# EyalMichaeli/SaSPA-Aug

Hardware: AMD Instinct MI355X
Metric: augmented images/sec (512x512, 50-step DDIM) (higher is better)
Workload: dtype bf16; 1 GPU; SD-v1.5 + Canny ControlNet, batch=8 512x512, 50 DDIM steps, CFG 7.5, ctrl-scale 0.75 (BASELINE.json configs[1]); step = Canny + CLIP + 50x(UNet+ControlNet) + VAE decode; batch_per_gpu=8, resolution=512, ddim_steps=50, weights=random-init, architecture-exact, parallelism=dp1 (image shards, one RCCL gather of the status vector), process_group=none (single process)

## Files before the change

### saspa-aug_amd/csrc/gemm_internal.h

```cpp
#pragma once
#include <hip/hip_runtime.h>

#include "saspa_hip.h"

__attribute__((visibility("hidden"))) int saspa_gemm_pp_launch(const SaspaGemmParams& p, hipStream_t s, int ksplit, int fn);
__attribute__((visibility("hidden"))) bool saspa_gemm_pp_eligible(const SaspaGemmParams& p);
__attribute__((visibility("hidden"))) int saspa_gemm_splitk_reduce(const SaspaGemmParams& p, hipStream_t s, int ksplit);
__attribute__((visibility("hidden"))) int saspa_gemm_npart8(const SaspaGemmParams& p, int BM, int BN, int G, int tiles);
static inline int saspa_balanced_grid(int tiles, int cap) {
  if (cap < 1) cap = 1;
  if (tiles <= cap) return tiles;
  const int rounds = (tiles + cap - 1) / cap;
  return (tiles + rounds - 1) / rounds;
}

__attribute__((visibility("hidden"))) int saspa_gemm_ws_launch(const SaspaGemmParams& p, hipStream_t s);
__attribute__((visibility("hidden"))) bool saspa_gemm_ws_eligible(const SaspaGemmParams& p);
__attribute__((visibility("hidden"))) int saspa_gemm_as_launch(const SaspaGemmParams& p, hipStream_t s);
__attribute__((visibility("hidden"))) bool saspa_gemm_as_ok(const SaspaGemmParams& p);
__attribute__((visibility("hidden"))) int saspa_gn_slabs(int c8);
```

### saspa-aug_amd/csrc/saspa_gemm_pp.hip

```cpp
#include <cstdlib>

#include "common.h"
#include "gemm_internal.h"

#ifndef SASPA_PP_CT_ABL
#define SASPA_PP_CT_ABL 0
#endif

namespace {

typedef bf16_t T;

__device__ __forceinline__ void mma(const u32x4& wf, const u32x4& xf, f32x4& acc) {
  acc = __builtin_amdgcn_mfma_f32_16x16x32_bf16(__builtin_bit_cast(bf16x8, wf), __builtin_bit_cast(bf16x8, xf), acc, 0, 0, 0);
}

template <int N> __device__ __forceinline__ void wait_vm() { asm volatile("s_waitcnt vmcnt(%0)" ::"n"(N) : "memory"); }

template <int FN, bool PW, bool UP, int LOOP>
__global__ __launch_bounds__(512) void gemm_pp_kernel(const SaspaGemmParams p, const int ntiles_abl, const int npart8) {
  constexpr bool ONEBAR = LOOP == 1;
  const int ntiles = ntiles_abl & 0x00ffffff;
#ifdef SASPA_GEMM_ABLATION
  const int abl = (ntiles_abl >> 28) & 15;
  const bool stamp = (ntiles_abl >> 27) & 1;
  unsigned long long st0 = 0, sr0 = 0, st1 = 0, sr1 = 0, sr_setup = 0, sr_issue = 0, sr_e0 = 0, sr_e1 = 0;
  const unsigned long long sr_entry = __builtin_amdgcn_s_memrealtime();
  const int eabl = (ntiles_abl >> 24) & 7;
#else
  constexpr int abl = SASPA_PP_CT_ABL, eabl = 0;
#endif
  constexpr int BM = 256, BN = 64 * FN, BK = 64, SZ = 2;
  constexpr int STAGE = (BM + BN) * 8;
  constexpr int CP = BN + 8;
  constexpr int EPI = 128 * CP * SZ / 16;
  constexpr int NLDS = 2 * STAGE > EPI ? 2 * STAGE : EPI;
  constexpr int NIMG = 4;
  constexpr int ADDV_F = (1 + 2 * NIMG) * BN;
  __shared__ u32x4 lds[NLDS + ADDV_F / 4];
  float* const addvb = reinterpret_cast<float*>(lds + NLDS);
  float* const addvr = addvb + BN;

  const int tid = threadIdx.x;
  const int lane = tid & 63;
  const int wave = __builtin_amdgcn_readfirstlane(tid >> 6);
  const int wm = wave >> 2, wn = wave & 3;
  const int frow = lane & 15, fg = lane >> 4;
  const int lr = lane >> 3;
  const int kcs = (lane & 7) ^ lr;

  const int nbn = (p.N + BN - 1) / BN;
  const int G = gridDim.x;
  int tile;
  {
    const int L = blockIdx.x;
    const int qd = G >> 3, rr = G & 7, xcd = L & 7, idx = L >> 3;
    tile = (xcd < rr ? xcd * (qd + 1) : rr * (qd + 1) + (xcd - rr) * qd) + idx;
  }
  const int z = blockIdx.z;
  const int i1 = z / p.nb2, i2 = z - i1 * p.nb2;
  const T* a0 = reinterpret_cast<const T*>(p.a0) + (i1 * p.sa1 + i2 * p.sa2);
  const T* a1 = reinterpret_cast<const T*>(p.a1);
  const T* w = reinterpret_cast<const T*>(p.w) + (i1 * p.sw1 + i2 * p.sw2);
  const long long ooff = i1 * p.so1 + i2 * p.so2;

  const int nk_all = (p.K + BK - 1) / BK;
  const int kt_per = (nk_all + gridDim.y - 1) / gridDim.y;
  const int kt0 = blockIdx.y * kt_per;
  const int nk = max(0, min(nk_all, kt0 + kt_per) - kt0);

  const int hw = p.hout * p.wout;
  const int ctot = p.c0 + p.c1;
  const int chunk_major = p.korder == SASPA_KORDER_CHUNK ? 1 : 0;
  const int hv = UP ? 2 * p.hin : p.hin, wv = UP ? 2 * p.win : p.win;
  const int back = (PW || UP) ? 0 : p.win + 1;
  const T* a0s = a0 - (long long)back * p.lda0;
  const T* a1s = p.c1 > 0 ? a1 - (long long)back * p.lda1 : a0s;
  auto make_desc = [](const T* base, bool live) __attribute__((always_inline)) {
    return __builtin_amdgcn_make_buffer_rsrc(const_cast<T*>(base), (short)0, live ? 0x7fffffff : 0, 0x00020000);
  };
  const rsrc_t rsn = make_desc(w, false);

  int bm = 0, bn = 0;
  int va[4], vb[PW ? 1 : 4], vc[UP ? 4 : 1];
  unsigned offb0 = 0;
  int nrows = 0;
  int ku = 0, cu = 0, dyu = 0, dxu = 0, staged = 0;
  int src = -1;
  const int arow0 = wm * 128 + (wave & 3) * 8 + lr;

  auto setup_tile = [&](int t) __attribute__((always_inline)) {
    if (npart8 > 0) {
      const int G8 = G >> 3;
      const int k = t / G, r = t - k * G;
      const int x = r / G8;
      const int q = k * G8 + (r - x * G8);
      bm = q / npart8;
      bn = x * npart8 + (q - bm * npart8);
    } else {
      bm = t / nbn;
      bn = t - bm * nbn;
    }
    if (!PW) {
      int m = bm * BM + arow0;
      int b = m / hw;
      int rem = m - b * hw;
      int oy = rem / p.wout;
      int ox = rem - oy * p.wout;
#pragma unroll
      for (int s = 0; s < 4; ++s) {
        const bool live = m < p.M;
        const int eb = live ? b : 0, ey = live ? oy : 0, ex = live ? ox : 0;
        const int iy0 = ey * p.stride - p.pad, ix0 = ex * p.stride - p.pad;
        if (UP) {
          va[s] = eb * p.hin * p.win;
          vc[UP ? s : 0] = ((iy0 + 1) << 16) | (ix0 + 1);
          int mask = 0;
          for (int ty = 0; ty < 3; ++ty)
            for (int tx = 0; tx < 3; ++tx)
              if ((unsigned)(iy0 + ty) < (unsigned)hv && (unsigned)(ix0 + tx) < (unsigned)wv) mask |= 1 << (ty * 3 + tx);
          vb[PW ? 0 : s] = mask;
        } else {
          int outside = 0;
#pragma unroll
          for (int tb = 0; tb < 9; ++tb) {
            if (tb == 4) continue;
            const int ty = tb / 3, tx = tb - ty * 3;
            if (!((unsigned)(iy0 + ty) < (unsigned)hv && (unsigned)(ix0 + tx) < (unsigned)wv)) outside |= 1 << (tb < 4 ? tb : tb - 1);
          }
          vb[PW ? 0 : s] = (eb * p.hin * p.win + (ey * p.stride) * p.win + ex * p.stride) | (outside << 24);
        }
        m += 32;
        ox += 32;
        while (ox >= p.wout) { ox -= p.wout; ++oy; }
        while (oy >= p.hout) { oy -= p.hout; ++b; }
      }
    }
    offb0 = (unsigned)((bn * BN + wave * 8 + lr) * p.ldw * SZ + kcs * 16);
    nrows = p.N - bn * BN;
    ku = kt0 * BK;
    if (chunk_major) {
      const int ntap = p.kh * p.kw;
      const int chunk = kt0 / ntap, tap = kt0 - chunk * ntap;
      cu = chunk * BK;
      dyu = tap / p.kw;
      dxu = tap - dyu * p.kw;
    } else {
      const int tapu = ku / ctot;
      cu = ku - tapu * ctot;
      dyu = tapu / p.kw;
      dxu = tapu - dyu * p.kw;
    }
    staged = 0;
    src = -1;
  };

  bool sv = false;
  rsrc_t rs = rsn, rswv = rsn;
  int ldsz = 0, soff = 0, soffw = 0, sdy = 0, sdx = 0, bsh = 0, tapbit = 0;
  unsigned amask = 0;
  auto begin_stage = [&]() __attribute__((always_inline)) {
    sv = staged < nk;
    const bool s0 = cu < p.c0;
    ldsz = (s0 ? p.lda0 : p.lda1) * SZ;
    rs = make_desc(s0 ? a0s : a1s, sv);
    rswv = make_desc(w, sv);
    soff = (s0 ? cu : cu - p.c0) * SZ;
    soffw = ku * SZ;
    if (!UP) {
      if (!ONEBAR && src != (s0 ? 0 : 1)) {
        src = s0 ? 0 : 1;
#pragma unroll
        for (int s = 0; s < 4; ++s) {
          int px;
          if (PW) {
            const int m = bm * BM + arow0 + 32 * s;
            px = m < p.M ? m : 0;
          } else {
            px = vb[PW ? 0 : s] & 0xffffff;
          }
          va[s] = (int)(__umul24((unsigned)px, (unsigned)ldsz) + (unsigned)(kcs * 16));
        }
      }
      if (!PW) {
        const int tb = dyu * 3 + dxu;
        soff += (dyu * p.win + dxu) * ldsz;
        bsh = 7 - (tb < 4 ? tb : tb - 1);
        amask = tb == 4 ? 0u : 0x80000000u;
      }
    } else {
      tapbit = dyu * 3 + dxu;
      sdy = dyu;
      sdx = dxu;
    }
    ++staged;
    ku += BK;
    const int cu_t = cu + BK;
    const int wc = (cu_t >= ctot) ? 1 : 0;
    const int dx1 = dxu + (chunk_major ? 1 : wc);
    const int wx = (dx1 == p.kw) ? 1 : 0;
    const int dy1 = dyu + wx;
    const int wy = (chunk_major && dy1 == p.kh) ? 1 : 0;
    cu = chunk_major ? cu + (wy ? BK : 0) : (wc ? cu_t - ctot : cu_t);
    dxu = wx ? 0 : dx1;
    dyu = wy ? 0 : dy1;
  };
  int cur = 0, oth = STAGE;
  const int swz0 = fg ^ (frow & 7);
  int ra0 = (wm * 128 + frow) * 8 + swz0, ra1 = ra0 ^ 4;
  int rb0 = (BM + wn * (16 * FN) + frow) * 8 + swz0, rb1 = rb0 ^ 4;
  const int dma_a = (wm * 128 + (wave & 3) * 8) * 8;
  const int dma_b = (BM + wave * 8) * 8;

  auto stage_a = [&](const int s, const int buf) __attribute__((always_inline)) {
    unsigned off;
    if (UP) {
      const int iy = ((vc[UP ? s : 0] >> 16) - 1 + sdy) >> 1, ix = ((vc[UP ? s : 0] & 0xffff) - 1 + sdx) >> 1;
      const int px = va[s] + iy * p.win + ix;
      const bool ok = ((vb[PW ? 0 : s] >> tapbit) & 1) != 0;
      off = ok ? __umul24((unsigned)px, (unsigned)ldsz) + (unsigned)(kcs * 16) : kInvalid;
    } else if (PW) {
      if (ONEBAR) {
        const int m = bm * BM + arow0 + 32 * s;
        off = __umul24((unsigned)(m < p.M ? m : 0), (unsigned)ldsz) + (unsigned)(kcs * 16);
      } else {
        off = (unsigned)va[s];
      }
    } else {
      const unsigned base = ONEBAR ? __umul24((unsigned)vb[PW ? 0 : s] & 0xffffffu, (unsigned)ldsz) + (unsigned)(kcs * 16) : (unsigned)va[s];
      off = (((unsigned)vb[PW ? 0 : s] << bsh) & amask) | base;
    }
    __builtin_amdgcn_raw_ptr_buffer_load_lds(rs, (lds_void_t*)(lds + buf + dma_a + s * 32 * 8), 16, (int)off, soff, 0, 0);
  };
  auto stage_b = [&](const int i, const int buf) __attribute__((always_inline)) {
    const bool ok = (wave + 8 * i) * 8 < nrows;
    __builtin_amdgcn_raw_ptr_buffer_load_lds(rswv, (lds_void_t*)(lds + buf + dma_b + i * 64 * 8), 16, (int)(ok ? offb0 : kInvalid),
                                             soffw + i * 64 * p.ldw * SZ, 0, 0);
  };
  auto stage_slice = [&](const int s, const int buf) __attribute__((always_inline)) {
    stage_a(s, buf);
    if (s < 3) {
      stage_b(s, buf);
    } else {
#pragma unroll
      for (int i = 3; i < FN; ++i) stage_b(i, buf);
    }
  };

  f32x4 acc[8][FN];
  u32x4 wb[FN][2], xa[2][2];
  int dbgv[4] = {0, 0, 0, 0};
#if defined(SASPA_GEMM_ABLATION) || SASPA_PP_CT_ABL
#pragma unroll
  for (int j = 0; j < FN; ++j) wb[j][0] = wb[j][1] = u32x4{(unsigned)j, 0u, 0x3f803f80u, 0x3f803f80u};
#pragma unroll
  for (int i = 0; i < 2; ++i) xa[i][0] = xa[i][1] = u32x4{(unsigned)i, 1u, 0x3f803f80u, 0x3f803f80u};
#endif

  auto phase = [&](const int P, const int SS, const int sbuf, const bool sync) __attribute__((always_inline)) {
    if (!(abl & 2)) {
      if (P == 0) {
#pragma unroll
        for (int j = 0; j < FN; ++j) {
          wb[j][0] = lds[rb0 + j * 16 * 8];
          wb[j][1] = lds[rb1 + j * 16 * 8];
        }
        __builtin_amdgcn_sched_barrier(0);
      }
#pragma unroll
      for (int i = 0; i < 2; ++i) {
        xa[i][0] = lds[ra0 + (P * 32 + i * 16) * 8];
        xa[i][1] = lds[ra1 + (P * 32 + i * 16) * 8];
      }
    }
    if (!(abl & 4)) stage_slice(SS, sbuf);
    if (sync && P == 3) wait_vm<6>();
    if (sync && P == 0) asm volatile("s_waitcnt lgkmcnt(4)" ::: "memory");
    if (sync && !(abl & 8)) __builtin_amdgcn_s_barrier();
    __builtin_amdgcn_s_setprio(1);
    if (abl & 1) {
#pragma unroll
      for (int i = 0; i < 2; ++i) { asm volatile("" ::"v"(xa[i][0])); asm volatile("" ::"v"(xa[i][1])); }
#pragma unroll
      for (int j = 0; j < FN; ++j) { asm volatile("" ::"v"(wb[j][0])); asm volatile("" ::"v"(wb[j][1])); }
    } else {
#pragma unroll
      for (int kk = 0; kk < 2; ++kk)
#pragma unroll
        for (int i = 0; i < 2; ++i)
#pragma unroll
          for (int j = 0; j < FN; ++j) mma(wb[j][kk], xa[i][kk], acc[P * 2 + i][j]);
    }
    __builtin_amdgcn_s_setprio(0);
    if (sync && !(abl & 8)) __builtin_amdgcn_s_barrier();
  };

  setup_tile(tile);
#ifdef SASPA_GEMM_ABLATION
  if (stamp) sr_setup = __builtin_amdgcn_s_memrealtime();
#endif
  for (;;) {
#pragma unroll
    for (int i = 0; i < 8; ++i)
#pragma unroll
      for (int j = 0; j < FN; ++j) acc[i][j] = f32x4{0.f, 0.f, 0.f, 0.f};

    if (gridDim.y == 1) {
      constexpr int PCS = BN / 64;
      const int nimg = p.rowvec ? NIMG : 1;
      for (int pc = wave; pc < PCS * (1 + 2 * NIMG); pc += 8) {
        const int rowi = pc / PCS, part = pc - rowi * PCS;
        const int voff = (bn * BN + part * 64 + lane) * 4;
        if (rowi == 0) {
          const rsrc_t rb = __builtin_amdgcn_make_buffer_rsrc(const_cast<float*>(p.bias), (short)0, p.bias ? p.N * 4 : 0, 0x00020000);
          __builtin_amdgcn_raw_ptr_buffer_load_lds(rb, (lds_void_t*)(addvb + part * 64), 4, voff, 0, 0, 0);
        } else {
          const int hi = rowi - 1, h = hi / NIMG, il = hi - h * NIMG;
          const int img = min(bm * BM + h * 128, p.M - 1) / hw + il;
          const bool live = p.rowvec && il < nimg && (long long)img * hw < p.M;
          const rsrc_t rr = __builtin_amdgcn_make_buffer_rsrc(const_cast<float*>(p.rowvec) + (live ? (long long)img * p.ldrv : 0), (short)0,
                                                              live ? p.N * 4 : 0, 0x00020000);
          __builtin_amdgcn_raw_ptr_buffer_load_lds(rr, (lds_void_t*)(addvr + hi * BN + part * 64), 4, voff, 0, 0, 0);
        }
      }
    }

    if (nk > 0) {
      if (ONEBAR) {
        constexpr int NB1 = (FN + 1) / 2;
        auto stage_p1 = [&](const int buf) __attribute__((always_inline)) {
          stage_a(0, buf);
#pragma unroll
          for (int i = 0; i < NB1; ++i) stage_b(i, buf);
        };
        auto stage_p2 = [&](const int buf) __attribute__((always_inline)) {
          stage_a(1, buf);
#pragma unroll
          for (int i = NB1; i < FN; ++i) stage_b(i, buf);
        };
        begin_stage();
#pragma unroll
        for (int s = 0; s < 4; ++s) stage_slice(s, cur);
        begin_stage();
        stage_p1(oth);
        stage_p2(oth);
        stage_a(2, oth);
        wait_vm<3 + FN>();
        __builtin_amdgcn_s_barrier();
#ifdef SASPA_GEMM_ABLATION
        if (stamp) { st0 = __builtin_amdgcn_s_memtime(); sr0 = __builtin_amdgcn_s_memrealtime(); }
#endif
        auto read_b = [&]() __attribute__((always_inline)) {
          const int o1 = rb0 ^ 4;
#pragma unroll
          for (int j = 0; j < FN; ++j) {
            wb[j][0] = lds[rb0 + j * 16 * 8];
            wb[j][1] = lds[o1 + j * 16 * 8];
          }
        };
        auto read_a = [&](const int P) __attribute__((always_inline)) {
          const int o1 = ra0 ^ 4;
#pragma unroll
          for (int i = 0; i < 2; ++i) {
            xa[i][0] = lds[ra0 + (P * 32 + i * 16) * 8];
            xa[i][1] = lds[o1 + (P * 32 + i * 16) * 8];
          }
        };
        auto mfma_block = [&](const int P) __attribute__((always_inline)) {
          if (abl & 1) {
#pragma unroll
            for (int i = 0; i < 2; ++i) { asm volatile("" ::"v"(xa[i][0])); asm volatile("" ::"v"(xa[i][1])); }
#pragma unroll
            for (int j = 0; j < FN; ++j) { asm volatile("" ::"v"(wb[j][0])); asm volatile("" ::"v"(wb[j][1])); }
            return;
          }
          __builtin_amdgcn_s_setprio(1);
#pragma unroll
          for (int kk = 0; kk < 2; ++kk)
#pragma unroll
            for (int i = 0; i < 2; ++i)
#pragma unroll
              for (int j = 0; j < FN; ++j) mma(wb[j][kk], xa[i][kk], acc[P * 2 + i][j]);
          __builtin_amdgcn_s_setprio(0);
        };
        auto swap_bufs = [&]() __attribute__((always_inline)) {
          const int d = oth - cur;
          ra0 += d; rb0 += d;
          cur += d;
          oth -= d;
        };
        if (wm != 0) { read_b(); read_a(0); }
#ifdef SASPA_GEMM_ABLATION
#define BAR() do { if (!(abl & 8)) __builtin_amdgcn_s_barrier(); } while (0)
#define RD(...) { if (!(abl & 2)) { __VA_ARGS__ } }
#define ST(...) { if (!(abl & 4)) { __VA_ARGS__ } }
#else
#define BAR() __builtin_amdgcn_s_barrier()
#define RD(...) { __VA_ARGS__ }
#define ST(...) { __VA_ARGS__ }
// ... 33 lines not shown
        if (stamp) { st1 = __builtin_amdgcn_s_memtime(); sr1 = __builtin_amdgcn_s_memrealtime(); }
#endif
      } else if (LOOP == 2) {
        auto stage_q1 = [&](const int buf) __attribute__((always_inline)) {
          stage_a(0, buf);
          stage_a(1, buf);
#pragma unroll
          for (int i = 0; i < FN; ++i) stage_b(i, buf);
        };
        auto read_a2 = [&](const int i, const int S) __attribute__((always_inline)) {
          xa[i][0] = lds[ra0 + (S * 32 + i * 16) * 8];
          xa[i][1] = lds[ra1 + (S * 32 + i * 16) * 8];
        };
        auto mma_row = [&](const int i, const int R) __attribute__((always_inline)) {
          if (abl & 1) {
            asm volatile("" ::"v"(xa[i][0])); asm volatile("" ::"v"(xa[i][1]));
#pragma unroll
            for (int j = 0; j < FN; ++j) { asm volatile("" ::"v"(wb[j][0])); asm volatile("" ::"v"(wb[j][1])); }
            return;
          }
#pragma unroll
          for (int kk = 0; kk < 2; ++kk)
#pragma unroll
            for (int j = 0; j < FN; ++j) mma(wb[j][kk], xa[i][kk], acc[R][j]);
        };
        int wsum[2] = {0, 0};
        long long tloop0 = 0;
        if (abl & 32) tloop0 = __builtin_amdgcn_s_memtime();
        auto qphase = [&](const int Q) __attribute__((always_inline)) {
          if (!(abl & 8)) __builtin_amdgcn_s_barrier();
          if (!(abl & 64)) __builtin_amdgcn_s_setprio(1);
          mma_row(0, 4 * Q + 0);
          __builtin_amdgcn_sched_barrier(0);
          if (!(abl & 2)) read_a2(0, 2 * Q + 1);
          __builtin_amdgcn_sched_barrier(0);
          mma_row(1, 4 * Q + 1);
          __builtin_amdgcn_sched_barrier(0);
          if (!(abl & 2)) read_a2(1, 2 * Q + 1);
          __builtin_amdgcn_sched_barrier(0);
          mma_row(0, 4 * Q + 2);
          mma_row(1, 4 * Q + 3);
          if (!(abl & 64)) __builtin_amdgcn_s_setprio(0);
          long long tb = 0;
          if (abl & 32) { __builtin_amdgcn_sched_barrier(0); tb = __builtin_amdgcn_s_memtime(); }
          if (!(abl & 8)) __builtin_amdgcn_s_barrier();
          if (abl & 32) {
            const long long te = __builtin_amdgcn_s_memtime();
            asm volatile("s_waitcnt lgkmcnt(0)" ::: "memory");
            wsum[Q] += (int)(te - tb);
            __builtin_amdgcn_sched_barrier(0);
          }
        };
        begin_stage();
#pragma unroll
        for (int s = 0; s < 4; ++s) stage_slice(s, cur);
        begin_stage();
        stage_q1(oth);
        wait_vm<2 + FN>();
        __builtin_amdgcn_s_barrier();
        if (wm == 1) __builtin_amdgcn_s_barrier();
#ifdef SASPA_GEMM_ABLATION
        if (stamp) { st0 = __builtin_amdgcn_s_memtime(); sr0 = __builtin_amdgcn_s_memrealtime(); }
#endif
        for (int t = 0; t < nk; ++t) {
          if (!(abl & 2)) {
#pragma unroll
            for (int j = 0; j < FN; ++j) {
              wb[j][0] = lds[rb0 + j * 16 * 8];
              wb[j][1] = lds[rb1 + j * 16 * 8];
            }
            __builtin_amdgcn_sched_barrier(0);
            read_a2(0, 0);
            read_a2(1, 0);
          }
          if (!(abl & 4)) { stage_a(2, oth); stage_a(3, oth); }
          wait_vm<4 + FN>();
          asm volatile("s_waitcnt lgkmcnt(4)" ::: "memory");
          qphase(0);
          begin_stage();
          if (!(abl & 2)) { read_a2(0, 2); read_a2(1, 2); }
          if (!(abl & 4)) stage_q1(cur);
          wait_vm<4 + FN>();
          qphase(1);
          const int d = oth - cur;
          ra0 += d; ra1 += d; rb0 += d; rb1 += d;
          cur += d;
          oth -= d;
        }
#ifdef SASPA_GEMM_ABLATION
        if (stamp) { st1 = __builtin_amdgcn_s_memtime(); sr1 = __builtin_amdgcn_s_memrealtime(); }
#endif
        if (wm == 0) __builtin_amdgcn_s_barrier();
        if ((abl & 32) && blockIdx.x == 0 && blockIdx.y == 0 && blockIdx.z == 0 && (wave & 3) == 0 && lane == 0) {
          dbgv[0] = wsum[0]; dbgv[1] = wsum[1]; dbgv[2] = (int)(__builtin_amdgcn_s_memtime() - tloop0); dbgv[3] = 2 * nk;
        }
      } else {
      begin_stage();
#pragma unroll
      for (int s = 0; s < 4; ++s) stage_slice(s, cur);
      begin_stage();
#pragma unroll
      for (int s = 0; s < 3; ++s) stage_slice(s, oth);
#ifdef SASPA_GEMM_ABLATION
      if (stamp) sr_issue = __builtin_amdgcn_s_memrealtime();
#endif
      wait_vm<6>();
      __builtin_amdgcn_s_barrier();
      if (wm == 1) __builtin_amdgcn_s_barrier();
#ifdef SASPA_GEMM_ABLATION
      if (stamp) { st0 = __builtin_amdgcn_s_memtime(); sr0 = __builtin_amdgcn_s_memrealtime(); }
#endif
      for (int t = 0; t < nk; ++t) {
        phase(0, 3, oth, true);
        begin_stage();
        phase(1, 0, cur, true);
        phase(2, 1, cur, true);
        phase(3, 2, cur, true);
        const int d = oth - cur;
        ra0 += d; ra1 += d; rb0 += d; rb1 += d;
        cur += d;
        oth -= d;
      }
#ifdef SASPA_GEMM_ABLATION
      if (stamp) { st1 = __builtin_amdgcn_s_memtime(); sr1 = __builtin_amdgcn_s_memrealtime(); }
#endif
      if (wm == 0) __builtin_amdgcn_s_barrier();
      }
      wait_vm<0>();
      if (cur != 0) {
        ra0 -= STAGE; ra1 -= STAGE; rb0 -= STAGE; rb1 -= STAGE;
        cur = 0;
        oth = STAGE;
      }
    }
    __syncthreads();

    const int cbm = bm, cbn = bn;
    const int next = tile + G;
    const bool has_next = next < ntiles;

    int etid = threadIdx.x;
    asm volatile("" : "+v"(etid));
    const int elane = etid & 63;
    const int ewave = __builtin_amdgcn_readfirstlane(etid >> 6);
    const int ewm = ewave >> 2, ewn = ewave & 3, efrow = elane & 15, efg = elane >> 4;
    T* out = reinterpret_cast<T*>(p.out) + ooff;
    const T* res = p.residual ? reinterpret_cast<const T*>(p.residual) + ooff : nullptr;
#ifdef SASPA_GEMM_ABLATION
    if (stamp) sr_e0 = __builtin_amdgcn_s_memrealtime();
#endif
    if (eabl == 2) {
#pragma unroll
      for (int i = 0; i < 8; ++i)
#pragma unroll
        for (int j = 0; j < FN; ++j) asm volatile("" ::"v"(acc[i][j]));
    } else if (gridDim.y > 1) {
      float* ws = p.workspace + (long long)blockIdx.y * p.M * p.N;
#pragma unroll
      for (int i = 0; i < 8; ++i) {
        const int m = cbm * BM + ewm * 128 + i * 16 + efrow;
        if (m >= p.M) continue;
#pragma unroll
        for (int j = 0; j < FN; ++j) {
          const int n = cbn * BN + ewn * (16 * FN) + j * 16 + efg * 4;
          if (n >= p.N) continue;
          *reinterpret_cast<float4*>(ws + (long long)m * p.N + n) =
              make_float4(acc[i][j][0], acc[i][j][1], acc[i][j][2], acc[i][j][3]);
        }
      }
    } else {
      T* ct = reinterpret_cast<T*>(lds);
      T* ctg = ct + ewm * (64 * CP);
      const int gtid = etid & 255;
      const int m0 = cbm * BM + ewm * 128;
      const int img0 = min(m0, p.M - 1) / hw;
      const int mnext = (img0 + 1) * hw;
      const bool multi = p.rowvec && m0 + 128 > mnext && mnext < p.M;
      const float* avb = addvb + ewn * (16 * FN) + efg * 4;
      const float* av = addvr + ewm * NIMG * BN + ewn * (16 * FN) + efg * 4;
      float4 add[FN];
#pragma unroll
      for (int j = 0; j < FN; ++j) {
        add[j] = *reinterpret_cast<const float4*>(avb + j * 16);
        const float4 r4 = *reinterpret_cast<const float4*>(av + j * 16);
        add[j].x += r4.x; add[j].y += r4.y; add[j].z += r4.z; add[j].w += r4.w;
      }
      const int gunit = p.gn_stats ? p.gn_unit : BN;
      const int nunits = BN / gunit;
      const int rgs = 256 / nunits;
      const int gu = gtid % nunits, grg = gtid / nunits;
      float gsm = 0.f, gsq = 0.f;
      constexpr int CPR = BN / 8;
#pragma unroll
      for (int qt = 0; qt < 2; ++qt) {
        if (!multi) {
#pragma unroll
          for (int i = 0; i < 4; ++i) {
#pragma unroll
            for (int j = 0; j < FN; ++j) {
              const f32x4& c = acc[qt * 4 + i][j];
              float v[4] = {c[0] + add[j].x, c[1] + add[j].y, c[2] + add[j].z, c[3] + add[j].w};
#pragma unroll
              for (int r = 0; r < 4; ++r) v[r] *= p.alpha;
              Elem<T>::store4(ctg + (i * 16 + efrow) * CP + ewn * (16 * FN) + j * 16 + efg * 4, v);
            }
          }
        } else if (hw >= 43) {
#pragma unroll
          for (int i = 0; i < 4; ++i) {
            const int m = m0 + (qt * 4 + i) * 16 + efrow;
            const int il = (m >= mnext ? 1 : 0) + (m >= mnext + hw ? 1 : 0) + (m >= mnext + 2 * hw ? 1 : 0);
            const float* avr = av + il * BN;
#pragma unroll
            for (int j = 0; j < FN; ++j) {
              float4 ad = *reinterpret_cast<const float4*>(avb + j * 16);
              const float4 r4 = *reinterpret_cast<const float4*>(avr + j * 16);
              ad.x += r4.x; ad.y += r4.y; ad.z += r4.z; ad.w += r4.w;
              const f32x4& c = acc[qt * 4 + i][j];
              float v[4] = {c[0] + ad.x, c[1] + ad.y, c[2] + ad.z, c[3] + ad.w};
#pragma unroll
              for (int r = 0; r < 4; ++r) v[r] *= p.alpha;
              Elem<T>::store4(ctg + (i * 16 + efrow) * CP + ewn * (16 * FN) + j * 16 + efg * 4, v);
            }
          }
        } else {
#pragma unroll
          for (int i = 0; i < 4; ++i) {
            const int m = m0 + (qt * 4 + i) * 16 + efrow;
            const float* rvd = p.rowvec + (long long)(min(m, p.M - 1) / hw) * p.ldrv;
#pragma unroll
            for (int j = 0; j < FN; ++j) {
              const int n = cbn * BN + ewn * (16 * FN) + j * 16 + efg * 4;
              float4 ad = *reinterpret_cast<const float4*>(avb + j * 16);
              if (n < p.N) {
                const float4 r4 = *reinterpret_cast<const float4*>(rvd + n);
                ad.x += r4.x; ad.y += r4.y; ad.z += r4.z; ad.w += r4.w;
              }
              const f32x4& c = acc[qt * 4 + i][j];
              float v[4] = {c[0] + ad.x, c[1] + ad.y, c[2] + ad.z, c[3] + ad.w};
#pragma unroll
              for (int r = 0; r < 4; ++r) v[r] *= p.alpha;
              Elem<T>::store4(ctg + (i * 16 + efrow) * CP + ewn * (16 * FN) + j * 16 + efg * 4, v);
            }
          }
        }
        lds_barrier();
        const int mq = m0 + qt * 64;
        if (p.act == SASPA_ACT_GEGLU) {
          if constexpr (FN == 5) {
            constexpr int CPG = 20;
            for (int q = gtid; q < 64 * CPG; q += 256) {
              const int row = q / CPG, ch = q - row * CPG;
              const int m = mq + row;
              if (m >= p.M) continue;
              const int sub = ch / 10, c10 = ch - sub * 10;
              float a[8], g[8];
              unpack8(*reinterpret_cast<const uint4*>(ctg + row * CP + sub * 160 + c10 * 8), a);
              unpack8(*reinterpret_cast<const uint4*>(ctg + row * CP + sub * 160 + 80 + c10 * 8), g);
#pragma unroll
              for (int e = 0; e < 8; ++e) a[e] = fast_gelu_mul(a[e], g[e]);
              *reinterpret_cast<uint4*>(out + (long long)m * p.ldo + cbn * 160 + ch * 8) = pack8(a);
            }
          }
        } else {
          auto finish = [&](u32x4 c4, const uint4 r4, const int row, const int ch, const int m, const int n) __attribute__((always_inline)) {
            if (res || p.act != SASPA_ACT_NONE) {
              float a[8];
              unpack8(__builtin_bit_cast(uint4, c4), a);
              if (p.act == SASPA_ACT_SILU) {
#pragma unroll
                for (int e = 0; e < 8; ++e) a[e] = a[e] * __builtin_amdgcn_rcpf(1.0f + __expf(-a[e]));
              } else if (p.act == SASPA_ACT_RELU) {
#pragma unroll
                for (int e = 0; e < 8; ++e) a[e] = fmaxf(a[e], 0.0f);
              }
              if (res) {
                float b[8];
                unpack8(r4, b);
#pragma unroll
                for (int e = 0; e < 8; ++e) a[e] += b[e];
              }
              if (p.act == SASPA_ACT_ADD_RELU) {
// ... 23 lines not shown
              if (res) {
#pragma unroll
                for (int k = 0; k < NB; ++k)
                  r4[k] = *reinterpret_cast<const uint4*>(res + (long long)(mq + row[k]) * p.ldr + cbn * BN + ch[k] * 8);
              }
#pragma unroll
              for (int k = 0; k < NB; ++k) {
                const u32x4 c4 = *reinterpret_cast<const u32x4*>(ctg + row[k] * CP + ch[k] * 8);
                finish(c4, r4[k], row[k], ch[k], mq + row[k], cbn * BN + ch[k] * 8);
              }
            }
          } else {
            for (int q = gtid; q < 64 * CPR; q += 256) {
              const int row = q / CPR, ch = q - row * CPR;
              const int m = mq + row, n = cbn * BN + ch * 8;
              if (m >= p.M || n >= p.N) continue;
              const u32x4 c4 = *reinterpret_cast<const u32x4*>(ctg + row * CP + ch * 8);
              uint4 r4 = make_uint4(0u, 0u, 0u, 0u);
              if (res) r4 = *reinterpret_cast<const uint4*>(res + (long long)m * p.ldr + n);
              finish(c4, r4, row, ch, m, n);
            }
          }
        }
#ifdef SASPA_GEMM_ABLATION
        if (stamp && qt == 0) sr_e1 = __builtin_amdgcn_s_memrealtime();
#endif
        if (p.gn_stats) {
          lds_barrier();
          const int nrows = min(64, p.M - mq);
          if (grg < rgs) {
            for (int r = grg; r < nrows; r += rgs) {
              const uint32_t* src = reinterpret_cast<const uint32_t*>(ctg + r * CP + gu * gunit);
              for (int j = 0; j < gunit; j += 2) {
                const bf16x2_t w2 = __builtin_bit_cast(bf16x2_t, src[j >> 1]);
                gsm = __builtin_amdgcn_fdot2_f32_bf16(w2, __builtin_bit_cast(bf16x2_t, 0x3F803F80u), gsm, false);
                gsq = __builtin_amdgcn_fdot2_f32_bf16(w2, w2, gsq, false);
              }
            }
          }
        }
        lds_barrier();
      }
      if (p.gn_stats) {
        float* scr = reinterpret_cast<float*>(ct + 128 * CP) + ewm * 512;
        if (grg < rgs) {
          scr[(grg * nunits + gu) * 2] = gsm;
          scr[(grg * nunits + gu) * 2 + 1] = gsq;
        }
        lds_barrier();
        if (gtid < nunits * 2 && m0 < p.M) {
          const int uu = gtid >> 1, k = gtid & 1;
          float a = 0.f;
          for (int g = 0; g < rgs; ++g) a += scr[(g * nunits + uu) * 2 + k];
          p.gn_stats[((long long)(cbm * 2 + ewm) * (p.N / p.gn_unit) + (cbn * BN) / p.gn_unit + uu) * 2 + k] = a;
        }
        lds_barrier();
      }
    }
#ifdef SASPA_GEMM_ABLATION
    if (stamp && etid == 0) {
      const unsigned long long sr_issued = __builtin_amdgcn_s_memrealtime();
      __threadfence();
      unsigned long long* o = reinterpret_cast<unsigned long long*>(reinterpret_cast<T*>(p.out) + (long long)p.M * p.ldo) + 16 * blockIdx.x;
      o[0] = sr0;
      o[1] = sr1;
      o[2] = ((st1 - st0) << 20) | ((sr0 - sr_entry) & 0xfffff);
      o[3] = __builtin_amdgcn_s_memrealtime();
      o[4] = sr_entry;
      o[5] = sr_setup;
      o[6] = sr_issue;
      o[7] = sr_e0;
      o[8] = sr_e1;
      o[9] = sr_issued;
    }
#endif
    if (!has_next) break;
    tile = next;
    setup_tile(tile);
  }
  if (abl & 32) {
    __syncthreads();
    if (blockIdx.x == 0 && blockIdx.y == 0 && blockIdx.z == 0 && (wave & 3) == 0 && lane == 0) {
      int* dbg = reinterpret_cast<int*>(p.out) + (wave >> 2) * 4;
      dbg[0] = dbgv[0]; dbg[1] = dbgv[1]; dbg[2] = dbgv[2]; dbg[3] = dbgv[3];
    }
  }
}

template <int FN, int ONEBAR>
int launch_pp(const SaspaGemmParams& p, hipStream_t s, int ksplit) {
  constexpr int BM = 256, BN = 64 * FN;
  const int tiles = ((p.N + BN - 1) / BN) * ((p.M + BM - 1) / BM);
  const int zy = ksplit * p.nb1 * p.nb2;
  const int gx = saspa_balanced_grid(tiles, 256 / zy);
  dim3 grid(gx, ksplit, p.nb1 * p.nb2);
  const bool pw = p.kh == 1 && p.kw == 1 && p.stride == 1 && p.pad == 0 && !p.upsample;
  static const int abl = getenv("SASPA_GEMM_ABLATE") ? (atoi(getenv("SASPA_GEMM_ABLATE")) & 15) : 0;
  static const int stamp = getenv("SASPA_GEMM_STAMP") ? (atoi(getenv("SASPA_GEMM_STAMP")) & 1) : 0;
  static const int eabl = getenv("SASPA_GEMM_EPI_ABLATE") ? (atoi(getenv("SASPA_GEMM_EPI_ABLATE")) & 7) : 0;
  const int ta = tiles | (abl << 28) | (stamp << 27) | (eabl << 24);
  const int npart8 = saspa_gemm_npart8(p, BM, BN, gx, tiles);
  if (pw) hipLaunchKernelGGL((gemm_pp_kernel<FN, true, false, ONEBAR>), grid, dim3(512), 0, s, p, ta, npart8);
  else if (p.upsample) hipLaunchKernelGGL((gemm_pp_kernel<FN, false, true, ONEBAR>), grid, dim3(512), 0, s, p, ta, npart8);
  else hipLaunchKernelGGL((gemm_pp_kernel<FN, false, false, ONEBAR>), grid, dim3(512), 0, s, p, ta, npart8);
  SASPA_CHECK_LAUNCH();
  if (ksplit > 1) return saspa_gemm_splitk_reduce(p, s, ksplit);
  return 0;
}

}

bool saspa_gemm_pp_eligible(const SaspaGemmParams& p) {
  const int ctot = p.c0 + p.c1;
  if (p.dtype != SASPA_BF16) return false;
  if (p.act == SASPA_ACT_GEGLU && ((p.N % 320) != 0 || p.residual || p.alpha != 1.0f)) return false;
  if ((ctot % 64) != 0 || (p.c1 > 0 && (p.c0 % 64) != 0)) return false;
  if ((p.N % 8) != 0 || (p.ldo % 8) != 0 || (p.residual && (p.ldr % 8) != 0)) return false;
  const bool pw = p.kh == 1 && p.kw == 1 && p.stride == 1 && p.pad == 0 && !p.upsample;
  if (!pw) {
    if (p.kh != 3 || p.kw != 3 || p.pad != 1) return false;
    const int hv = p.upsample ? 2 * p.hin : p.hin, wv = p.upsample ? 2 * p.win : p.win;
    if ((p.hout - 1) * p.stride > hv - 1 || (p.wout - 1) * p.stride > wv - 1) return false;
    if (p.upsample && (p.hin >= 16000 || p.win >= 16000)) return false;
  }
  if ((long long)p.batch * p.hin * p.win >= (1ll << 24) || p.M >= (1 << 24)) return false;
  if ((long long)p.lda0 * 2 >= (1ll << 24) || (long long)p.lda1 * 2 >= (1ll << 24)) return false;
  return true;
}

int saspa_gemm_pp_launch(const SaspaGemmParams& p, hipStream_t s, int ksplit, int fn) {
  if (fn == 4 || fn == 5) {
    const char* e = getenv("SASPA_GEMM_PP_LOOP");
    const int loop = e ? atoi(e) : 2;
#ifdef SASPA_GEMM_ABLATION
    if (loop == 1) fn += 10;
#endif
    if (loop != 0 && loop != 1) fn += 20;
#ifndef SASPA_GEMM_ABLATION
    if (loop == 1) fn += 20;
#endif
  }
  if (fn == 5) return launch_pp<5, 0>(p, s, ksplit);
  if (fn == 4) return launch_pp<4, 0>(p, s, ksplit);
#ifdef SASPA_GEMM_ABLATION
  if (fn == 15) return launch_pp<5, 1>(p, s, ksplit);
  if (fn == 14) return launch_pp<4, 1>(p, s, ksplit);
#endif
  if (fn == 25) return launch_pp<5, 2>(p, s, ksplit);
  if (fn == 24) return launch_pp<4, 2>(p, s, ksplit);
  return SASPA_ERANGE;
}
```

Before: 7.158 images/s.

## Precompute GEMM tile setup on host and overlap first-stage loads with setup

```diff
diff --git a/saspa-aug_amd/csrc/gemm_internal.h b/saspa-aug_amd/csrc/gemm_internal.h
--- a/saspa-aug_amd/csrc/gemm_internal.h
+++ b/saspa-aug_amd/csrc/gemm_internal.h
@@ -1,7 +1,12 @@
 #pragma once
+#ifndef SASPA_PP_SETUP_HOST_TEST
 #include <hip/hip_runtime.h>
+#endif
+#include <stdint.h>
 
 #include "saspa_hip.h"
+
+#ifndef SASPA_PP_SETUP_HOST_TEST
 
 __attribute__((visibility("hidden"))) int saspa_gemm_pp_launch(const SaspaGemmParams& p, hipStream_t s, int ksplit, int fn);
 __attribute__((visibility("hidden"))) bool saspa_gemm_pp_eligible(const SaspaGemmParams& p);
@@ -19,3 +24,127 @@
 __attribute__((visibility("hidden"))) int saspa_gemm_as_launch(const SaspaGemmParams& p, hipStream_t s);
 __attribute__((visibility("hidden"))) bool saspa_gemm_as_ok(const SaspaGemmParams& p);
 __attribute__((visibility("hidden"))) int saspa_gn_slabs(int c8);
+#endif
+
+#ifdef __HIPCC__
+#define SASPA_PP_HD __host__ __device__ __forceinline__
+#else
+#define SASPA_PP_HD inline
+#endif
+
+struct PpDiv {
+  uint32_t mul, sh;
+};
+constexpr uint32_t kPpDivLimit = 1u << 24;
+
+inline bool pp_div_make(long long d, PpDiv* o) {
+  if (d < 1 || d >= (long long)kPpDivLimit) return false;
+  uint32_t l = 0;
+  while ((1ll << l) < d) ++l;
+  o->mul = (uint32_t)(((1ull << (24 + l)) + (uint64_t)d - 1) / (uint64_t)d);
+  o->sh = l;
+  return true;
+}
+SASPA_PP_HD uint32_t pp_div(uint32_t n, const PpDiv d) { return (uint32_t)(((uint64_t)(n << 8) * d.mul) >> 32) >> d.sh; }
+
+struct PpSetup {
+  PpDiv d_hw, d_wout, d_nbn, d_g, d_g8, d_np8, d_nb2, d_ntap, d_kw, d_ct;
+  PpDiv d_nunits, d_gnu;
+  int gunit, nunits, rgs, nun;
+  int nbn;
+  int g, g8, np8;
+  int nb2;
+  int nk_all, kt_per;
+  int hw, wout, ctot, ct;
+  int ntap, kw;
+  int hv, wv;
+  int hwin, swin;
+  int lda0b, lda1b, ldwb, ldw64b;
+  long long back0b, back1b;
+};
+
+inline int pp_setup_fill(const SaspaGemmParams& p, int bn, int gx, int gy, int npart8, long long tiles, PpSetup* s) {
+  const long long lim = kPpDivLimit;
+  if (bn < 64 || gx < 1 || gy < 1 || npart8 < 0 || tiles < 1 || tiles >= lim) return SASPA_ERANGE;
+  if (p.M < 1 || p.M >= lim || p.N < 1 || (long long)p.N + bn >= lim || p.K < 1 || p.K >= (1 << 30)) return SASPA_ERANGE;
+  if (p.gn_stats && (p.gn_unit < 1 || p.gn_unit > bn)) return SASPA_ERANGE;
+  const bool pw = p.kh == 1 && p.kw == 1 && p.stride == 1 && p.pad == 0 && !p.upsample;
+  const long long hw = (long long)p.hout * p.wout, ctot = (long long)p.c0 + p.c1, ntap = (long long)p.kh * p.kw;
+  const long long nk_all = ((long long)p.K + 63) / 64, kt_per = (nk_all + gy - 1) / gy;
+  if (kt_per * gy >= lim || (ctot % 64) != 0 || (long long)p.nb1 * p.nb2 >= 65536) return SASPA_ERANGE;
+  if (npart8 > 0 && (gx & 7)) return SASPA_ERANGE;
+  const long long hwin = (long long)p.hin * p.win, swin = (long long)p.stride * p.win;
+  if (hwin >= lim || swin >= lim || (long long)p.lda0 * 2 >= lim || (long long)p.lda1 * 2 >= lim || (long long)p.ldw * 128 > 0x7fffffffll)
+    return SASPA_ERANGE;
+  s->nbn = (p.N + bn - 1) / bn;
+  s->g = gx;
+  s->g8 = gx >> 3;
+  s->np8 = npart8;
+  s->nb2 = p.nb2;
+  if (!pp_div_make(hw, &s->d_hw) || !pp_div_make(p.wout, &s->d_wout) || !pp_div_make(s->nbn, &s->d_nbn) ||
+      !pp_div_make(gx, &s->d_g) || !pp_div_make(s->g8 > 0 ? s->g8 : 1, &s->d_g8) || !pp_div_make(npart8 > 0 ? npart8 : 1, &s->d_np8) ||
+      !pp_div_make(p.nb2, &s->d_nb2) || !pp_div_make(ntap, &s->d_ntap) || !pp_div_make(p.kw, &s->d_kw) ||
+      !pp_div_make(ctot / 64, &s->d_ct))
+    return SASPA_ERANGE;
+  s->gunit = p.gn_stats ? p.gn_unit : bn;
+  s->nunits = bn / s->gunit;
+  s->rgs = 256 / s->nunits;
+  s->nun = p.gn_stats ? p.N / p.gn_unit : 0;
+  if (!pp_div_make(s->nunits, &s->d_nunits) || !pp_div_make(p.gn_stats ? p.gn_unit : 1, &s->d_gnu)) return SASPA_ERANGE;
+  s->nk_all = (int)nk_all;
+  s->kt_per = (int)kt_per;
+  s->hw = (int)hw;
+  s->wout = p.wout;
+  s->ctot = (int)ctot;
+  s->ct = (int)(ctot / 64);
+  s->ntap = (int)ntap;
+  s->kw = p.kw;
+  s->hv = p.upsample ? 2 * p.hin : p.hin;
+  s->wv = p.upsample ? 2 * p.win : p.win;
+  s->hwin = (int)hwin;
+  s->swin = (int)swin;
+  s->lda0b = p.lda0 * 2;
+  s->lda1b = p.lda1 * 2;
+  s->ldwb = p.ldw * 2;
+  s->ldw64b = p.ldw * 128;
+  const long long back = (pw || p.upsample) ? 0 : p.win + 1;
+  s->back0b = back * p.lda0 * 2;
+  s->back1b = back * p.lda1 * 2;
+  return 0;
+}
+
+SASPA_PP_HD void pp_tile_to_block(const PpSetup& s, int t, int* bm, int* bn) {
+  if (s.np8 > 0) {
+    const int k = (int)pp_div((uint32_t)t, s.d_g), r = t - k * s.g;
+    const int x = (int)pp_div((uint32_t)r, s.d_g8);
+    const int q = k * s.g8 + (r - x * s.g8);
+    *bm = (int)pp_div((uint32_t)q, s.d_np8);
+    *bn = x * s.np8 + (q - *bm * s.np8);
+  } else {
+    *bm = (int)pp_div((uint32_t)t, s.d_nbn);
+    *bn = t - *bm * s.nbn;
+  }
+}
+SASPA_PP_HD void pp_row_to_pixel(const PpSetup& s, int m, int* b, int* oy, int* ox) {
+  *b = (int)pp_div((uint32_t)m, s.d_hw);
+  const int rem = m - *b * s.hw;
+  *oy = (int)pp_div((uint32_t)rem, s.d_wout);
+  *ox = rem - *oy * s.wout;
+}
+SASPA_PP_HD void pp_kstart(const PpSetup& s, bool chunk_major, int kt0, int* cu, int* dyu, int* dxu) {
+  int tap;
+  if (chunk_major) {
+    const int chunk = (int)pp_div((uint32_t)kt0, s.d_ntap);
+    tap = kt0 - chunk * s.ntap;
+    *cu = chunk * 64;
+  } else {
+    tap = (int)pp_div((uint32_t)kt0, s.d_ct);
+    *cu = (kt0 - tap * s.ct) * 64;
+  }
+  *dyu = (int)pp_div((uint32_t)tap, s.d_kw);
+  *dxu = tap - *dyu * s.kw;
+}
+SASPA_PP_HD void pp_z_to_batch(const PpSetup& s, int z, int* i1, int* i2) {
+  *i1 = (int)pp_div((uint32_t)z, s.d_nb2);
+  *i2 = z - *i1 * s.nb2;
+}
diff --git a/saspa-aug_amd/csrc/saspa_gemm_pp.hip b/saspa-aug_amd/csrc/saspa_gemm_pp.hip
--- a/saspa-aug_amd/csrc/saspa_gemm_pp.hip
+++ b/saspa-aug_amd/csrc/saspa_gemm_pp.hip
@@ -18,7 +18,7 @@
 template <int N> __device__ __forceinline__ void wait_vm() { asm volatile("s_waitcnt vmcnt(%0)" ::"n"(N) : "memory"); }
 
 template <int FN, bool PW, bool UP, int LOOP>
-__global__ __launch_bounds__(512) void gemm_pp_kernel(const SaspaGemmParams p, const int ntiles_abl, const int npart8) {
+__global__ __launch_bounds__(512) void gemm_pp_kernel(const PpSetup su_arg, const SaspaGemmParams p, const int ntiles_abl, const int npart8) {
   constexpr bool ONEBAR = LOOP == 1;
   const int ntiles = ntiles_abl & 0x00ffffff;
 #ifdef SASPA_GEMM_ABLATION
@@ -49,33 +49,39 @@
   const int lr = lane >> 3;
   const int kcs = (lane & 7) ^ lr;
 
-  const int nbn = (p.N + BN - 1) / BN;
-  const int G = gridDim.x;
+  PpSetup su;
+  auto load_su = [&]() __attribute__((always_inline)) {
+    typedef const __attribute__((address_space(4))) uint32_t* ka_t;
+    ka_t ka = (ka_t)__builtin_amdgcn_kernarg_segment_ptr();
+    asm volatile("" : "+s"(ka));
+    uint32_t* const d = reinterpret_cast<uint32_t*>(&su);
+    static_assert(sizeof(PpSetup) % 4 == 0, "copied by dwords");
+#pragma unroll
+    for (unsigned i = 0; i < sizeof(PpSetup) / 4; ++i) d[i] = ka[i];
+  };
+  (void)su_arg;
+  load_su();
   int tile;
   {
     const int L = blockIdx.x;
+    const int G = su.g;
     const int qd = G >> 3, rr = G & 7, xcd = L & 7, idx = L >> 3;
     tile = (xcd < rr ? xcd * (qd + 1) : rr * (qd + 1) + (xcd - rr) * qd) + idx;
   }
   const int z = blockIdx.z;
-  const int i1 = z / p.nb2, i2 = z - i1 * p.nb2;
+  int i1, i2;
+  pp_z_to_batch(su, z, &i1, &i2);
   const T* a0 = reinterpret_cast<const T*>(p.a0) + (i1 * p.sa1 + i2 * p.sa2);
   const T* a1 = reinterpret_cast<const T*>(p.a1);
   const T* w = reinterpret_cast<const T*>(p.w) + (i1 * p.sw1 + i2 * p.sw2);
   const long long ooff = i1 * p.so1 + i2 * p.so2;
 
-  const int nk_all = (p.K + BK - 1) / BK;
-  const int kt_per = (nk_all + gridDim.y - 1) / gridDim.y;
-  const int kt0 = blockIdx.y * kt_per;
-  const int nk = max(0, min(nk_all, kt0 + kt_per) - kt0);
-
-  const int hw = p.hout * p.wout;
-  const int ctot = p.c0 + p.c1;
+  const int kt0 = blockIdx.y * su.kt_per;
+  const int nk = max(0, min(su.nk_all, kt0 + su.kt_per) - kt0);
+
   const int chunk_major = p.korder == SASPA_KORDER_CHUNK ? 1 : 0;
-  const int hv = UP ? 2 * p.hin : p.hin, wv = UP ? 2 * p.win : p.win;
-  const int back = (PW || UP) ? 0 : p.win + 1;
-  const T* a0s = a0 - (long long)back * p.lda0;
-  const T* a1s = p.c1 > 0 ? a1 - (long long)back * p.lda1 : a0s;
+  const T* a0s = reinterpret_cast<const T*>(reinterpret_cast<const char*>(a0) - su.back0b);
+  const T* a1s = p.c1 > 0 ? reinterpret_cast<const T*>(reinterpret_cast<const char*>(a1) - su.back1b) : a0s;
   auto make_desc = [](const T* base, bool live) __attribute__((always_inline)) {
     return __builtin_amdgcn_make_buffer_rsrc(const_cast<T*>(base), (short)0, live ? 0x7fffffff : 0, 0x00020000);
   };
@@ -89,36 +95,32 @@
   int src = -1;
   const int arow0 = wm * 128 + (wave & 3) * 8 + lr;
 
-  auto setup_tile = [&](int t) __attribute__((always_inline)) {
-    if (npart8 > 0) {
-      const int G8 = G >> 3;
-      const int k = t / G, r = t - k * G;
-      const int x = r / G8;
-      const int q = k * G8 + (r - x * G8);
-      bm = q / npart8;
-      bn = x * npart8 + (q - bm * npart8);
-    } else {
-      bm = t / nbn;
-      bn = t - bm * nbn;
-    }
+  auto setup_scalar = [&](int t) __attribute__((always_inline)) {
+    pp_tile_to_block(su, t, &bm, &bn);
+    offb0 = (unsigned)((bn * BN + wave * 8 + lr) * su.ldwb + kcs * 16);
+    nrows = p.N - bn * BN;
+    ku = kt0 * BK;
+    pp_kstart(su, chunk_major != 0, kt0, &cu, &dyu, &dxu);
+    staged = 0;
+    src = -1;
+  };
+  auto setup_lanes = [&]() __attribute__((always_inline)) {
     if (!PW) {
       int m = bm * BM + arow0;
-      int b = m / hw;
-      int rem = m - b * hw;
-      int oy = rem / p.wout;
-      int ox = rem - oy * p.wout;
+      int b, oy, ox;
+      pp_row_to_pixel(su, m < p.M ? m : 0, &b, &oy, &ox);
 #pragma unroll
       for (int s = 0; s < 4; ++s) {
         const bool live = m < p.M;
         const int eb = live ? b : 0, ey = live ? oy : 0, ex = live ? ox : 0;
         const int iy0 = ey * p.stride - p.pad, ix0 = ex * p.stride - p.pad;
         if (UP) {
-          va[s] = eb * p.hin * p.win;
+          va[s] = eb * su.hwin;
           vc[UP ? s : 0] = ((iy0 + 1) << 16) | (ix0 + 1);
           int mask = 0;
           for (int ty = 0; ty < 3; ++ty)
             for (int tx = 0; tx < 3; ++tx)
-              if ((unsigned)(iy0 + ty) < (unsigned)hv && (unsigned)(ix0 + tx) < (unsigned)wv) mask |= 1 << (ty * 3 + tx);
+              if ((unsigned)(iy0 + ty) < (unsigned)su.hv && (unsigned)(ix0 + tx) < (unsigned)su.wv) mask |= 1 << (ty * 3 + tx);
           vb[PW ? 0 : s] = mask;
         } else {
           int outside = 0;
@@ -126,33 +128,16 @@
           for (int tb = 0; tb < 9; ++tb) {
             if (tb == 4) continue;
             const int ty = tb / 3, tx = tb - ty * 3;
-            if (!((unsigned)(iy0 + ty) < (unsigned)hv && (unsigned)(ix0 + tx) < (unsigned)wv)) outside |= 1 << (tb < 4 ? tb : tb - 1);
-          }
-          vb[PW ? 0 : s] = (eb * p.hin * p.win + (ey * p.stride) * p.win + ex * p.stride) | (outside << 24);
+            if (!((unsigned)(iy0 + ty) < (unsigned)su.hv && (unsigned)(ix0 + tx) < (unsigned)su.wv)) outside |= 1 << (tb < 4 ? tb : tb - 1);
+          }
+          vb[PW ? 0 : s] = (eb * su.hwin + ey * su.swin + ex * p.stride) | (outside << 24);
         }
         m += 32;
         ox += 32;
-        while (ox >= p.wout) { ox -= p.wout; ++oy; }
+        while (ox >= su.wout) { ox -= su.wout; ++oy; }
         while (oy >= p.hout) { oy -= p.hout; ++b; }
       }
     }
-    offb0 = (unsigned)((bn * BN + wave * 8 + lr) * p.ldw * SZ + kcs * 16);
-    nrows = p.N - bn * BN;
-    ku = kt0 * BK;
-    if (chunk_major) {
-      const int ntap = p.kh * p.kw;
-      const int chunk = kt0 / ntap, tap = kt0 - chunk * ntap;
-      cu = chunk * BK;
-      dyu = tap / p.kw;
-      dxu = tap - dyu * p.kw;
-    } else {
-      const int tapu = ku / ctot;
-      cu = ku - tapu * ctot;
-      dyu = tapu / p.kw;
-      dxu = tapu - dyu * p.kw;
-    }
-    staged = 0;
-    src = -1;
   };
 
   bool sv = false;
@@ -162,7 +147,7 @@
   auto begin_stage = [&]() __attribute__((always_inline)) {
     sv = staged < nk;
     const bool s0 = cu < p.c0;
-    ldsz = (s0 ? p.lda0 : p.lda1) * SZ;
+    ldsz = s0 ? su.lda0b : su.lda1b;
     rs = make_desc(s0 ? a0s : a1s, sv);
     rswv = make_desc(w, sv);
     soff = (s0 ? cu : cu - p.c0) * SZ;
@@ -196,12 +181,12 @@
     ++staged;
     ku += BK;
     const int cu_t = cu + BK;
-    const int wc = (cu_t >= ctot) ? 1 : 0;
+    const int wc = (cu_t >= su.ctot) ? 1 : 0;
     const int dx1 = dxu + (chunk_major ? 1 : wc);
     const int wx = (dx1 == p.kw) ? 1 : 0;
     const int dy1 = dyu + wx;
     const int wy = (chunk_major && dy1 == p.kh) ? 1 : 0;
-    cu = chunk_major ? cu + (wy ? BK : 0) : (wc ? cu_t - ctot : cu_t);
+    cu = chunk_major ? cu + (wy ? BK : 0) : (wc ? cu_t - su.ctot : cu_t);
     dxu = wx ? 0 : dx1;
     dyu = wy ? 0 : dy1;
   };
@@ -235,7 +220,7 @@
   auto stage_b = [&](const int i, const int buf) __attribute__((always_inline)) {
     const bool ok = (wave + 8 * i) * 8 < nrows;
     __builtin_amdgcn_raw_ptr_buffer_load_lds(rswv, (lds_void_t*)(lds + buf + dma_b + i * 64 * 8), 16, (int)(ok ? offb0 : kInvalid),
-                                             soffw + i * 64 * p.ldw * SZ, 0, 0);
+                                             soffw + i * su.ldw64b, 0, 0);
   };
   auto stage_slice = [&](const int s, const int buf) __attribute__((always_inline)) {
     stage_a(s, buf);
@@ -295,36 +280,60 @@
     if (sync && !(abl & 8)) __builtin_amdgcn_s_barrier();
   };
 
-  setup_tile(tile);
-#ifdef SASPA_GEMM_ABLATION
-  if (stamp) sr_setup = __builtin_amdgcn_s_memrealtime();
-#endif
+  auto zero_acc = [&]() __attribute__((always_inline)) {
+    __builtin_amdgcn_sched_barrier(0);
+#pragma unroll
+    for (int i = 0; i < 8; ++i)
+#pragma unroll
+      for (int j = 0; j < FN; ++j) acc[i][j] = f32x4{0.f, 0.f, 0.f, 0.f};
+  };
   for (;;) {
-#pragma unroll
-    for (int i = 0; i < 8; ++i)
-#pragma unroll
-      for (int j = 0; j < FN; ++j) acc[i][j] = f32x4{0.f, 0.f, 0.f, 0.f};
+    setup_scalar(tile);
+    if (nk > 0) {
+      rswv = make_desc(w, true);
+      soffw = ku * SZ;
+#pragma unroll
+      for (int i = 0; i < FN; ++i) stage_b(i, cur);
+    }
+    __builtin_amdgcn_sched_barrier(0);
+    setup_lanes();
+#ifdef SASPA_GEMM_ABLATION
+    if (stamp) sr_setup = __builtin_amdgcn_s_memrealtime();
+#endif
+    if (nk > 0) {
+      begin_stage();
+#pragma unroll
+      for (int s = 0; s < 4; ++s) stage_a(s, cur);
+    }
 
     if (gridDim.y == 1) {
       constexpr int PCS = BN / 64;
-      const int nimg = p.rowvec ? NIMG : 1;
-      for (int pc = wave; pc < PCS * (1 + 2 * NIMG); pc += 8) {
-        const int rowi = pc / PCS, part = pc - rowi * PCS;
-        const int voff = (bn * BN + part * 64 + lane) * 4;
-        if (rowi == 0) {
-          const rsrc_t rb = __builtin_amdgcn_make_buffer_rsrc(const_cast<float*>(p.bias), (short)0, p.bias ? p.N * 4 : 0, 0x00020000);
-          __builtin_amdgcn_raw_ptr_buffer_load_lds(rb, (lds_void_t*)(addvb + part * 64), 4, voff, 0, 0, 0);
-        } else {
-          const int hi = rowi - 1, h = hi / NIMG, il = hi - h * NIMG;
-          const int img = min(bm * BM + h * 128, p.M - 1) / hw + il;
-          const bool live = p.rowvec && il < nimg && (long long)img * hw < p.M;
-          const rsrc_t rr = __builtin_amdgcn_make_buffer_rsrc(const_cast<float*>(p.rowvec) + (live ? (long long)img * p.ldrv : 0), (short)0,
-                                                              live ? p.N * 4 : 0, 0x00020000);
-          __builtin_amdgcn_raw_ptr_buffer_load_lds(rr, (lds_void_t*)(addvr + hi * BN + part * 64), 4, voff, 0, 0, 0);
-        }
-      }
-    }
-
+      static_assert(NIMG == 4 && 2 * NIMG == 8, "rows 0 .. 7: one per wave");
+      auto row_desc = [&](const int rowi) __attribute__((always_inline)) {
+        const int hi = max(rowi - 1, 0), h = hi >> 2, il = hi & 3;
+        const int img = (int)pp_div((uint32_t)min(bm * BM + h * 128, p.M - 1), su.d_hw) + il;
+        const bool rv = p.rowvec && (long long)img * su.hw < p.M;
+        const bool live = rowi == 0 ? p.bias != nullptr : rv;
+        const float* base = rowi == 0 ? p.bias : p.rowvec + (rv ? (long long)img * p.ldrv : 0);
+        const unsigned long long ba = reinterpret_cast<unsigned long long>(base);
+        const unsigned blo = __builtin_amdgcn_readfirstlane((unsigned)ba), bhi = __builtin_amdgcn_readfirstlane((unsigned)(ba >> 32));
+        const int nrec = __builtin_amdgcn_readfirstlane(live ? p.N * 4 : 0);
+        return __builtin_amdgcn_make_buffer_rsrc(reinterpret_cast<float*>(((unsigned long long)bhi << 32) | blo), (short)0, nrec, 0x00020000);
+      };
+      const int voff = (bn * BN + lane) * 4;
+      {
+        const rsrc_t rd = row_desc(wave);
+#pragma unroll
+        for (int part = 0; part < PCS; ++part)
+          __builtin_amdgcn_raw_ptr_buffer_load_lds(rd, (lds_void_t*)(addvb + wave * BN + part * 64), 4, voff + part * 256, 0, 0, 0);
+      }
+      if (wave < PCS) {
+        const rsrc_t rd = row_desc(2 * NIMG);
+        __builtin_amdgcn_raw_ptr_buffer_load_lds(rd, (lds_void_t*)(addvb + 2 * NIMG * BN + wave * 64), 4, voff + wave * 256, 0, 0, 0);
+      }
+    }
+
+    if (nk == 0) zero_acc();
     if (nk > 0) {
       if (ONEBAR) {
         constexpr int NB1 = (FN + 1) / 2;
@@ -339,12 +348,10 @@
           for (int i = NB1; i < FN; ++i) stage_b(i, buf);
         };
         begin_stage();
-#pragma unroll
-        for (int s = 0; s < 4; ++s) stage_slice(s, cur);
-        begin_stage();
         stage_p1(oth);
         stage_p2(oth);
         stage_a(2, oth);
+        zero_acc();
         wait_vm<3 + FN>();
         __builtin_amdgcn_s_barrier();
 #ifdef SASPA_GEMM_ABLATION
@@ -484,10 +491,11 @@
           }
         };
         begin_stage();
-#pragma unroll
-        for (int s = 0; s < 4; ++s) stage_slice(s, cur);
-        begin_stage();
         stage_q1(oth);
+#ifdef SASPA_GEMM_ABLATION
+        if (stamp) sr_issue = __builtin_amdgcn_s_memrealtime();
+#endif
+        zero_acc();
         wait_vm<2 + FN>();
         __builtin_amdgcn_s_barrier();
         if (wm == 1) __builtin_amdgcn_s_barrier();
@@ -529,13 +537,11 @@
       } else {
       begin_stage();
 #pragma unroll
-      for (int s = 0; s < 4; ++s) stage_slice(s, cur);
-      begin_stage();
-#pragma unroll
       for (int s = 0; s < 3; ++s) stage_slice(s, oth);
 #ifdef SASPA_GEMM_ABLATION
       if (stamp) sr_issue = __builtin_amdgcn_s_memrealtime();
 #endif
+      zero_acc();
       wait_vm<6>();
       __builtin_amdgcn_s_barrier();
       if (wm == 1) __builtin_amdgcn_s_barrier();
@@ -567,8 +573,10 @@
     }
     __syncthreads();
 
+    load_su();
+    const int hw = su.hw;
     const int cbm = bm, cbn = bn;
-    const int next = tile + G;
+    const int next = tile + su.g;
     const bool has_next = next < ntiles;
 
     int etid = threadIdx.x;
@@ -605,7 +613,7 @@
       T* ctg = ct + ewm * (64 * CP);
       const int gtid = etid & 255;
       const int m0 = cbm * BM + ewm * 128;
-      const int img0 = min(m0, p.M - 1) / hw;
+      const int img0 = (int)pp_div((uint32_t)min(m0, p.M - 1), su.d_hw);
       const int mnext = (img0 + 1) * hw;
       const bool multi = p.rowvec && m0 + 128 > mnext && mnext < p.M;
       const float* avb = addvb + ewn * (16 * FN) + efg * 4;
@@ -617,10 +625,8 @@
         const float4 r4 = *reinterpret_cast<const float4*>(av + j * 16);
         add[j].x += r4.x; add[j].y += r4.y; add[j].z += r4.z; add[j].w += r4.w;
       }
-      const int gunit = p.gn_stats ? p.gn_unit : BN;
-      const int nunits = BN / gunit;
-      const int rgs = 256 / nunits;
-      const int gu = gtid % nunits, grg = gtid / nunits;
+      const int gunit = su.gunit, nunits = su.nunits, rgs = su.rgs;
+      const int grg = (int)pp_div((uint32_t)gtid, su.d_nunits), gu = gtid - grg * nunits;
       float gsm = 0.f, gsq = 0.f;
       constexpr int CPR = BN / 8;
 #pragma unroll
@@ -659,7 +665,7 @@
 #pragma unroll
           for (int i = 0; i < 4; ++i) {
             const int m = m0 + (qt * 4 + i) * 16 + efrow;
-            const float* rvd = p.rowvec + (long long)(min(m, p.M - 1) / hw) * p.ldrv;
+            const float* rvd = p.rowvec + (long long)pp_div((uint32_t)min(m, p.M - 1), su.d_hw) * p.ldrv;
 #pragma unroll
             for (int j = 0; j < FN; ++j) {
               const int n = cbn * BN + ewn * (16 * FN) + j * 16 + efg * 4;
@@ -789,7 +795,7 @@
           const int uu = gtid >> 1, k = gtid & 1;
           float a = 0.f;
           for (int g = 0; g < rgs; ++g) a += scr[(g * nunits + uu) * 2 + k];
-          p.gn_stats[((long long)(cbm * 2 + ewm) * (p.N / p.gn_unit) + (cbn * BN) / p.gn_unit + uu) * 2 + k] = a;
+          p.gn_stats[((long long)(cbm * 2 + ewm) * su.nun + (int)pp_div((uint32_t)(cbn * BN), su.d_gnu) + uu) * 2 + k] = a;
         }
         lds_barrier();
       }
@@ -813,7 +819,6 @@
 #endif
     if (!has_next) break;
     tile = next;
-    setup_tile(tile);
   }
   if (abl & 32) {
     __syncthreads();
@@ -837,9 +842,11 @@
   static const int eabl = getenv("SASPA_GEMM_EPI_ABLATE") ? (atoi(getenv("SASPA_GEMM_EPI_ABLATE")) & 7) : 0;
   const int ta = tiles | (abl << 28) | (stamp << 27) | (eabl << 24);
   const int npart8 = saspa_gemm_npart8(p, BM, BN, gx, tiles);
-  if (pw) hipLaunchKernelGGL((gemm_pp_kernel<FN, true, false, ONEBAR>), grid, dim3(512), 0, s, p, ta, npart8);
-  else if (p.upsample) hipLaunchKernelGGL((gemm_pp_kernel<FN, false, true, ONEBAR>), grid, dim3(512), 0, s, p, ta, npart8);
-  else hipLaunchKernelGGL((gemm_pp_kernel<FN, false, false, ONEBAR>), grid, dim3(512), 0, s, p, ta, npart8);
+  PpSetup su;
+  if (const int rc = pp_setup_fill(p, BN, gx, ksplit, npart8, tiles, &su)) return rc;
+  if (pw) hipLaunchKernelGGL((gemm_pp_kernel<FN, true, false, ONEBAR>), grid, dim3(512), 0, s, su, p, ta, npart8);
+  else if (p.upsample) hipLaunchKernelGGL((gemm_pp_kernel<FN, false, true, ONEBAR>), grid, dim3(512), 0, s, su, p, ta, npart8);
+  else hipLaunchKernelGGL((gemm_pp_kernel<FN, false, false, ONEBAR>), grid, dim3(512), 0, s, su, p, ta, npart8);
   SASPA_CHECK_LAUNCH();
   if (ksplit > 1) return saspa_gemm_splitk_reduce(p, s, ksplit);
   return 0;
```

Measured after the change: 7.168 images/s, median of 6. About the same (+0.1%).
